# yisol/IDM-VTON

Measured on NVIDIA H100. Metric: try-on images/sec @768x1024, 30 steps, CFG 2.0, higher is better.
Workload: dtype fp16

## Files before the change

idm-vton_b200/csrc/gemm.cu:

```cuda
#include "gemm_common.cuh"
#include "host.h"
#include "wgmma.cuh"

namespace vton {

enum : int { KIND_F16 = 0, KIND_F16IN_F32OUT = 1, KIND_TF32 = 2 };

template <int BN, int STAGES, bool SC>
struct SmemLayout {
  static constexpr int B_BYTES = BN * 128;
  static constexpr int STAGE_BYTES = A_BYTES + B_BYTES;
  static constexpr int LDS = BN + 4;
  static constexpr int STG_BYTES = 128 * LDS * 4;
  static constexpr int RING = STAGES * STAGE_BYTES;
  static constexpr int STG_TOTAL = (SC ? 2 : 1) * STG_BYTES;
  static constexpr int BAR_OFFSET = RING > STG_TOTAL ? RING : STG_TOTAL;
  static constexpr int TOTAL = BAR_OFFSET + 256 + 1024;
};

constexpr int GEMM_THREADS = 288;

template <int BN, int STAGES, bool GEGLU, bool SC, int KIND>
__global__ void __launch_bounds__(GEMM_THREADS, 1)
gemm_conv_kernel(const __grid_constant__ CUtensorMap tmA, const __grid_constant__ CUtensorMap tmB,
                 const __grid_constant__ CUtensorMap tmS0, const __grid_constant__ CUtensorMap tmS1,
                 const __grid_constant__ CUtensorMap tmBs, const GemmParams p) {
  using L = SmemLayout<BN, STAGES, SC>;
  constexpr int KBK = KIND == KIND_TF32 ? 32 : 64;
  extern __shared__ uint8_t smem_raw[];
  const uint32_t smem_base = (smem_u32(smem_raw) + 1023u) & ~1023u;
  float* stg = reinterpret_cast<float*>(smem_raw + (smem_base - smem_u32(smem_raw)));
  const uint32_t bar_base = smem_base + L::BAR_OFFSET;
  auto full_bar = [&](int s) { return bar_base + 8u * s; };
  auto empty_bar = [&](int s) { return bar_base + 8u * (STAGES + s); };

  const int warp = threadIdx.x >> 5;
  const int lane = threadIdx.x & 31;
  const int tile = blockIdx.x;
  const int n_tile = tile % p.n_tiles;
  const int m_tile = tile / p.n_tiles;
  const int n0 = n_tile * BN;
  const int total_slabs = p.slabs_main + (SC ? p.slabs_sc : 0);

  int b0 = 0, y0 = 0, x0 = 0;
  if (p.conv) {
    const int tx = m_tile % p.tiles_x;
    const int ty = (m_tile / p.tiles_x) % p.tiles_y;
    const int tb = m_tile / (p.tiles_x * p.tiles_y);
    x0 = tx * p.bw;
    y0 = ty * p.bh;
    b0 = tb * p.bb;
  }

  if (warp == 8 && lane == 0) {
    tma_prefetch_desc(&tmA);
    tma_prefetch_desc(&tmB);
    if (SC) {
      tma_prefetch_desc(&tmS0);
      tma_prefetch_desc(&tmS1);
      tma_prefetch_desc(&tmBs);
    }
    for (int s = 0; s < STAGES; ++s) {
      mbar_init(full_bar(s), 1);
      mbar_init(empty_bar(s), 2);
    }
    fence_barrier_init();
  }
  pdl_wait();
  __syncthreads();
  pdl_launch_dependents();

  if (warp == 8) {
    if (lane == 0) {
      for (int s = 0; s < total_slabs; ++s) {
        const int stage = s % STAGES;
        const uint32_t phase = (s / STAGES) & 1;
        mbar_wait(empty_bar(stage), phase ^ 1);
        const uint32_t a_dst = smem_base + stage * L::STAGE_BYTES;
        const uint32_t b_dst = a_dst + A_BYTES;
        mbar_expect_tx(full_bar(stage), L::STAGE_BYTES);
        if (s < p.slabs_main) {
          if (p.conv) {
            const int tap = s / p.cin_slabs;
            const int c0 = (s - tap * p.cin_slabs) * KBK;
            const int dy = tap / 3 - 1, dx = tap % 3 - 1;
            tma_load_4d(a_dst, &tmA, full_bar(stage), c0, x0 * p.stride + dx, y0 * p.stride + dy, b0);
            tma_load_2d(b_dst, &tmB, full_bar(stage), c0, tap * p.cout + n0);
          } else {
            tma_load_2d(a_dst, &tmA, full_bar(stage), s * KBK, m_tile * BM);
            tma_load_2d(b_dst, &tmB, full_bar(stage), s * KBK, n0);
          }
        } else {
          const int ss = s - p.slabs_main;
          if (ss < p.sc_split)
            tma_load_4d(a_dst, &tmS0, full_bar(stage), ss * BK, x0, y0, b0);
          else
            tma_load_4d(a_dst, &tmS1, full_bar(stage), (ss - p.sc_split) * BK, x0, y0, b0);
          tma_load_2d(b_dst, &tmBs, full_bar(stage), ss * BK, n0);
        }
      }
    }
    return;
  }

  const int wg = warp >> 2;
  float acc[BN / 2];
  float acc_sc[BN / 2];
  auto run_slabs = [&](float (&accr)[BN / 2], int s_begin, int s_end) {
    for (int s = s_begin; s < s_end; ++s) {
      const int stage = s % STAGES;
      mbar_wait(full_bar(stage), (s / STAGES) & 1);
      const uint32_t a_src = smem_base + stage * L::STAGE_BYTES + wg * (64 * 128);
      const uint32_t b_src = smem_base + stage * L::STAGE_BYTES + A_BYTES;
      wgmma_fence();
#pragma unroll
      for (int k = 0; k < 4; ++k) {
        const uint64_t da = make_gmma_desc_sw128(a_src + k * 32, 0, 1024);
        const uint64_t db = make_gmma_desc_sw128(b_src + k * 32, 0, 1024);
        const int scale_d = (s > s_begin || k > 0) ? 1 : 0;
        if constexpr (KIND == KIND_TF32) {
          WgmmaTF32SS<BN>::mma(accr, da, db, scale_d);
        } else {
          WgmmaF16SS<BN, 0>::mma(accr, da, db, scale_d);
        }
      }
      wgmma_commit();
      wgmma_wait<1>();
      if (s > 0 && (threadIdx.x & 127) == 0) mbar_arrive(empty_bar((s - 1) % STAGES));
    }
  };
  run_slabs(acc, 0, p.slabs_main);
  if constexpr (SC) run_slabs(acc_sc, p.slabs_main, total_slabs);
  wgmma_wait<0>();
  fence_regs(acc);
  if (SC) fence_regs(acc_sc);

  named_bar_sync(1, 256);
  {
    const int r0 = wg * 64 + ((warp & 3) << 4) + (lane >> 2);
    const int cq = (lane & 3) * 2;
#pragma unroll
    for (int i = 0; i < BN / 8; ++i) {
      *reinterpret_cast<float2*>(stg + r0 * L::LDS + i * 8 + cq) = make_float2(acc[4 * i], acc[4 * i + 1]);
      *reinterpret_cast<float2*>(stg + (r0 + 8) * L::LDS + i * 8 + cq) = make_float2(acc[4 * i + 2], acc[4 * i + 3]);
      if (SC) {
        float* s2 = stg + 128 * L::LDS;
        *reinterpret_cast<float2*>(s2 + r0 * L::LDS + i * 8 + cq) = make_float2(acc_sc[4 * i], acc_sc[4 * i + 1]);
        *reinterpret_cast<float2*>(s2 + (r0 + 8) * L::LDS + i * 8 + cq) = make_float2(acc_sc[4 * i + 2], acc_sc[4 * i + 3]);
      }
    }
  }
  named_bar_sync(1, 256);
  const int row = threadIdx.x & 127;
  const int half = threadIdx.x >> 7;
  long long out_row;
  int sample;
  map_row(p, m_tile, row, &out_row, &sample);
  const float* srow = stg + row * L::LDS;
  if (KIND == KIND_F16) {
    epilogue_store<BN, GEGLU>(p, srow, SC ? srow + 128 * L::LDS : nullptr, n_tile, out_row, sample, half, 2);
    return;
  }
  if (out_row < 0) return;
  const float* res_row = p.res_f32 ? p.res_f32 + out_row * p.N : nullptr;
#pragma unroll 1
  for (int c = half; c < BN / 32; c += 2) {
    const int ncol = n0 + c * 32;
    if (ncol >= p.N) continue;
#pragma unroll
    for (int g = 0; g < 8; ++g) {
      float4 v = *reinterpret_cast<const float4*>(srow + c * 32 + g * 4);
      if (p.bias_f32 != nullptr) {
        const float4 b4 = __ldg(reinterpret_cast<const float4*>(p.bias_f32 + ncol + g * 4));
        v.x += b4.x, v.y += b4.y, v.z += b4.z, v.w += b4.w;
      }
      if (res_row != nullptr) {
        const float4 r4 = __ldg(reinterpret_cast<const float4*>(res_row + ncol + g * 4));
        v.x += r4.x, v.y += r4.y, v.z += r4.z, v.w += r4.w;
      }
      *reinterpret_cast<float4*>(p.out_f32 + out_row * p.N + ncol + g * 4) = v;
    }
  }
}

template <int BN, int STAGES, bool GEGLU, bool SC, int KIND>
static int launch_variant(const CUtensorMap& tmA, const CUtensorMap& tmB, const CUtensorMap& tmS0,
                          const CUtensorMap& tmS1, const CUtensorMap& tmBs, const GemmParams& p, int grid,
                          cudaStream_t stream) {
  using L = SmemLayout<BN, STAGES, SC>;
  static_assert(L::TOTAL <= 227 * 1024, "shared memory budget");
  auto kern = gemm_conv_kernel<BN, STAGES, GEGLU, SC, KIND>;
  static bool configured = false;
  if (!configured) {
    VTON_CUDA(cudaFuncSetAttribute(kern, cudaFuncAttributeMaxDynamicSharedMemorySize, L::TOTAL));
    configured = true;
  }
  VTON_CUDA(launch_kernel(kern, dim3(grid), dim3(GEMM_THREADS), L::TOTAL, stream, tmA, tmB, tmS0, tmS1, tmBs, p));
  count_launch();
  return kOk;
}

void set_auto_v2(int) {}
void set_cluster4(int) {}

static int pick_bn(int N, int m_tiles, bool geglu, bool has_shortcut, int force_bn) {
  if (force_bn >= 2000) force_bn -= 2000;
  else if (force_bn >= 1000) force_bn -= 1000;
  auto usable = [&](int bn) {
    if (geglu && ((bn != 256 && bn != 128) || N % bn != 0)) return false;
    if (has_shortcut && bn > 128) return false;
    return true;
  };
  if (force_bn) {
    const bool known = force_bn == 64 || force_bn == 128 || force_bn == 160 || force_bn == 192 || force_bn == 256;
    return known && usable(force_bn) ? force_bn : 0;
  }
  const int sms = num_sms();
  const int cands[5] = {256, 192, 160, 128, 64};
  double best = 1e300;
  int best_bn = 0;
  for (int bn : cands) {
    if (!usable(bn)) continue;
    if (bn != 128 && N % bn != 0 && !(bn == 64 && N < 64)) continue;
    const long long tiles = static_cast<long long>(m_tiles) * cdiv(N, bn);
    const long long waves = (tiles + sms - 1) / sms;
    const double cost = static_cast<double>(waves) * (bn + 64);
    if (cost < best * 0.999) {
      best = cost;
      best_bn = bn;
    }
  }
  return best_bn ? best_bn : 128;
}

static int dispatch(int bn, bool geglu, const CUtensorMap& tmA, const CUtensorMap& tmB, const CUtensorMap& tmS0,
                    const CUtensorMap& tmS1, const CUtensorMap& tmBs, GemmParams& p, int m_tiles,
                    cudaStream_t stream) {
  p.n_tiles = cdiv(p.N, bn);
  const int grid = m_tiles * p.n_tiles;
  if (geglu) {
    if (bn == 128) return launch_variant<128, 6, true, false, KIND_F16>(tmA, tmB, tmS0, tmS1, tmBs, p, grid, stream);
    if (bn == 256) return launch_variant<256, 4, true, false, KIND_F16>(tmA, tmB, tmS0, tmS1, tmBs, p, grid, stream);
    set_last_error("GEGLU epilogue supports BN 128/256 only (got %d)", bn);
    return kErrUnsupported;
  }
  if (p.slabs_sc) {
    if (bn == 64) return launch_variant<64, 8, false, true, KIND_F16>(tmA, tmB, tmS0, tmS1, tmBs, p, grid, stream);
    if (bn == 128) return launch_variant<128, 6, false, true, KIND_F16>(tmA, tmB, tmS0, tmS1, tmBs, p, grid, stream);
    set_last_error("shortcut epilogue supports BN 64/128 only (got %d)", bn);
    return kErrUnsupported;
  }
  switch (bn) {
    case 64: return launch_variant<64, 8, false, false, KIND_F16>(tmA, tmB, tmS0, tmS1, tmBs, p, grid, stream);
    case 128: return launch_variant<128, 6, false, false, KIND_F16>(tmA, tmB, tmS0, tmS1, tmBs, p, grid, stream);
    case 160: return launch_variant<160, 5, false, false, KIND_F16>(tmA, tmB, tmS0, tmS1, tmBs, p, grid, stream);
    case 192: return launch_variant<192, 4, false, false, KIND_F16>(tmA, tmB, tmS0, tmS1, tmBs, p, grid, stream);
    case 256: return launch_variant<256, 4, false, false, KIND_F16>(tmA, tmB, tmS0, tmS1, tmBs, p, grid, stream);
  }
  set_last_error("unsupported BN %d", bn);
  return kErrUnsupported;
}

int gemm_f16_impl(const void* A, long long lda, const void* W, long long ldw, void* out, long long ldo, int M, int N,
                  int K, const void* bias, const void* residual, long long ldr, const void* rowvec, long long ld_rowvec,
                  int rows_per_sample, int flags, int force_bn, cudaStream_t stream) {
  const int geglu = flags & 1;
  VTON_CHECK_ARG(M > 0 && N > 0 && K > 0, "gemm: empty problem M=%d N=%d K=%d", M, N, K);
  VTON_CHECK_ARG(K % 64 == 0, "gemm: K=%d must be a multiple of 64", K);
  VTON_CHECK_ARG(N % 8 == 0 && lda % 8 == 0 && ldw % 8 == 0 && ldo % 8 == 0, "gemm: N/lda/ldw/ldo must be multiples of 8");
  VTON_CHECK_ARG(!geglu || (N % 16 == 0 && !residual && !rowvec), "gemm: bad GEGLU configuration");
  VTON_CHECK_ARG(aligned_to(out, 16) && aligned_to(bias, 16) && aligned_to(residual, 16) && aligned_to(rowvec, 16),
                 "gemm: out/bias/residual/rowvec must be 16-byte aligned");
  VTON_CHECK_ARG((!residual || ldr % 8 == 0) && (!rowvec || ld_rowvec % 8 == 0),
                 "gemm: ldr=%lld / ld_rowvec=%lld must be multiples of 8", ldr, ld_rowvec);
  const int bn = pick_bn(N, cdiv(M, BM), geglu != 0, false, force_bn);
  VTON_CHECK_ARG(bn != 0, "gemm: tile width force_bn=%d unsupported for this problem (N=%d, geglu=%d)", force_bn, N, geglu);
  VTON_CHECK_ARG(!geglu || N % bn == 0, "gemm: GEGLU needs N %% BN == 0 (N=%d, BN=%d)", N, bn);
  CUtensorMap tmA, tmB;
  {
    uint64_t dims[2] = {static_cast<uint64_t>(K), static_cast<uint64_t>(M)};
    uint64_t strides[1] = {static_cast<uint64_t>(lda) * 2};
    uint32_t box[2] = {64, 128};
    if (int e = encode_tmap_f16(&tmA, A, 2, dims, strides, box)) return e;
  }
  {
    uint64_t dims[2] = {static_cast<uint64_t>(K), static_cast<uint64_t>(N)};
    uint64_t strides[1] = {static_cast<uint64_t>(ldw) * 2};
    uint32_t box[2] = {64, static_cast<uint32_t>(bn)};
    if (int e = encode_tmap_f16(&tmB, W, 2, dims, strides, box)) return e;
  }
  GemmParams p{};
  p.out = static_cast<__half*>(out);
  p.ld_out = static_cast<int>(ldo);
  p.M = M;
  p.N = N;
  p.bias = static_cast<const __half*>(bias);
  p.residual = static_cast<const __half*>(residual);
  p.ld_res = static_cast<int>(ldr);
  p.rowvec = static_cast<const __half*>(rowvec);
  p.ld_rowvec = static_cast<int>(ld_rowvec);
  p.rows_per_sample = rows_per_sample;
  p.slabs_main = K / 64;
  p.act_gelu = (flags & 4) ? 2 : ((flags & 2) ? 1 : 0);
  return dispatch(bn, geglu != 0, tmA, tmB, tmA, tmA, tmB, p, cdiv(M, BM), stream);
}

static void pick_box(int B, int H, int W, int* bw, int* bh, int* bb) {
  int w = 1;
  while (w < 128 && W % (w * 2) == 0) w *= 2;
  int h = 1;
  while (w * h < 128 && h * 2 <= H) h *= 2;
  *bw = w;
  *bh = h;
  *bb = 128 / (w * h);
  (void)B;
}

static int encode_nhwc(CUtensorMap* tm, const void* base, int B, int H, int W, int C, int ldc, int bw, int bh, int bb,
                       int pixel_step = 1) {
  uint64_t dims[4] = {static_cast<uint64_t>(C), static_cast<uint64_t>(W), static_cast<uint64_t>(H),
                      static_cast<uint64_t>(B)};
  uint64_t strides[3] = {static_cast<uint64_t>(ldc) * 2, static_cast<uint64_t>(W) * ldc * 2,
                         static_cast<uint64_t>(H) * W * ldc * 2};
  uint32_t box[4] = {64, static_cast<uint32_t>(bw * pixel_step), static_cast<uint32_t>(bh * pixel_step),
                     static_cast<uint32_t>(bb)};
  uint32_t estr[4] = {1, static_cast<uint32_t>(pixel_step), static_cast<uint32_t>(pixel_step), 1};
  return encode_tmap_f16(tm, base, 4, dims, strides, box, pixel_step > 1 ? estr : nullptr);
}

int conv3x3_impl(const void* x, long long ldx, int B, int Hin, int Win, int Cin, const void* w, int Cout, const void* bias,
                 const void* temb, long long ld_temb, const void* sc0, int C0, const void* sc1, int C1, const void* w_sc,
                 const void* bias_sc, const void* residual, long long ldr, void* out, long long ldo, int force_bn,
                 int stride, cudaStream_t stream) {
  VTON_CHECK_ARG(B > 0 && Hin > 0 && Win > 0, "conv3x3: empty input");
  VTON_CHECK_ARG(stride == 1 || stride == 2, "conv3x3: stride %d unsupported", stride);
  VTON_CHECK_ARG(stride == 1 || (!w_sc && !residual), "conv3x3: stride 2 has no shortcut / residual form");
  const int H = (Hin - 1) / stride + 1, W = (Win - 1) / stride + 1;
  VTON_CHECK_ARG(Cin % 64 == 0, "conv3x3: Cin=%d must be a multiple of 64 (pad channels)", Cin);
  VTON_CHECK_ARG(Cout % 8 == 0 && ldo % 8 == 0 && ldx % 8 == 0, "conv3x3: Cout/ldo/ldx must be multiples of 8");
  VTON_CHECK_ARG(C0 % 64 == 0 && C1 % 64 == 0, "conv3x3: shortcut source channels must be multiples of 64");
// ... 29 lines not shown
    }
    const int Csc = C0 + (sc1 ? C1 : 0);
    uint64_t dims[2] = {static_cast<uint64_t>(Csc), static_cast<uint64_t>(Cout)};
    uint64_t strides[1] = {static_cast<uint64_t>(Csc) * 2};
    uint32_t box[2] = {64, static_cast<uint32_t>(bn)};
    if (int e = encode_tmap_f16(&tmBs, w_sc, 2, dims, strides, box)) return e;
    p.slabs_sc = Csc / 64;
    p.sc_split = C0 / 64;
  }
  p.out = static_cast<__half*>(out);
  p.ld_out = static_cast<int>(ldo);
  p.M = B * H * W;
  p.N = Cout;
  p.bias = static_cast<const __half*>(bias);
  p.bias_sc = static_cast<const __half*>(bias_sc);
  p.residual = static_cast<const __half*>(residual);
  p.ld_res = static_cast<int>(ldr);
  p.rowvec = static_cast<const __half*>(temb);
  p.ld_rowvec = static_cast<int>(ld_temb);
  p.slabs_main = 9 * (Cin / 64);
  p.conv = 1;
  p.stride = stride;
  p.H = H;
  p.W = W;
  p.B = B;
  p.bw = bw;
  p.bh = bh;
  p.bb = bb;
  p.tiles_x = W / bw;
  p.tiles_y = cdiv(H, bh);
  p.cin_slabs = Cin / 64;
  p.cout = Cout;
  const int m_tiles = p.tiles_x * p.tiles_y * cdiv(B, bb);
  return dispatch(bn, false, tmA, tmB, tmS0, tmS1, tmBs, p, m_tiles, stream);
}

int conv3x3_f32_impl(const void* x, int B, int H, int W, int Cin, const void* w, int Cout, const void* bias,
                     const void* residual, void* out, int in_fp16, cudaStream_t stream) {
  VTON_CHECK_ARG(B > 0 && H > 0 && W > 0, "conv3x3_f32: empty input");
  VTON_CHECK_ARG(Cin % 32 == 0 && Cout % 32 == 0 && Cout >= 64, "conv3x3_f32: Cin=%d / Cout=%d must be multiples of 32 (Cout >= 64)", Cin, Cout);
  VTON_CHECK_ARG(!in_fp16 || Cin % 64 == 0, "conv3x3_f32: fp16 operands need Cin=%d to be a multiple of 64", Cin);
  VTON_CHECK_ARG(x && w && out, "conv3x3_f32: null pointer");
  const int esz = in_fp16 ? 2 : 4;
  const int bk = in_fp16 ? 64 : 32;
  int bw, bh, bb;
  pick_box(B, H, W, &bw, &bh, &bb);
  VTON_CHECK_ARG(bw * bh * bb == 128 && bw >= 8, "conv3x3_f32: W=%d H=%d cannot be tiled into 128-pixel boxes", W, H);
  const int m_tiles = (W / bw) * cdiv(H, bh) * cdiv(B, bb);
  const int bn = pick_bn(Cout, m_tiles, false, false, Cout % 256 == 0 ? 256 : 128);
  CUtensorMap tmA, tmB;
  {
    uint64_t dims[4] = {static_cast<uint64_t>(Cin), static_cast<uint64_t>(W), static_cast<uint64_t>(H), static_cast<uint64_t>(B)};
    uint64_t strides[3] = {static_cast<uint64_t>(Cin) * esz, static_cast<uint64_t>(W) * Cin * esz,
                           static_cast<uint64_t>(H) * W * Cin * esz};
    uint32_t box[4] = {static_cast<uint32_t>(bk), static_cast<uint32_t>(bw), static_cast<uint32_t>(bh), static_cast<uint32_t>(bb)};
    if (int e = in_fp16 ? encode_tmap_f16(&tmA, x, 4, dims, strides, box) : encode_tmap_f32(&tmA, x, 4, dims, strides, box)) return e;
  }
  {
    uint64_t dims[2] = {static_cast<uint64_t>(Cin), static_cast<uint64_t>(9) * Cout};
    uint64_t strides[1] = {static_cast<uint64_t>(Cin) * esz};
    uint32_t box[2] = {static_cast<uint32_t>(bk), static_cast<uint32_t>(bn)};
    if (int e = in_fp16 ? encode_tmap_f16(&tmB, w, 2, dims, strides, box) : encode_tmap_f32(&tmB, w, 2, dims, strides, box)) return e;
  }
  GemmParams p{};
  p.out_f32 = static_cast<float*>(out);
  p.bias_f32 = static_cast<const float*>(bias);
  p.res_f32 = static_cast<const float*>(residual);
  p.M = B * H * W;
  p.N = Cout;
  p.slabs_main = 9 * (Cin / bk);
  p.conv = 1;
  p.stride = 1;
  p.H = H;
  p.W = W;
  p.B = B;
  p.bw = bw;
  p.bh = bh;
  p.bb = bb;
  p.tiles_x = W / bw;
  p.tiles_y = cdiv(H, bh);
  p.cin_slabs = Cin / bk;
  p.cout = Cout;
  p.n_tiles = cdiv(Cout, bn);
  const int grid = m_tiles * p.n_tiles;
  if (in_fp16) {
    if (bn == 256) return launch_variant<256, 4, false, false, KIND_F16IN_F32OUT>(tmA, tmB, tmA, tmA, tmB, p, grid, stream);
    return launch_variant<128, 6, false, false, KIND_F16IN_F32OUT>(tmA, tmB, tmA, tmA, tmB, p, grid, stream);
  }
  if (bn == 256) return launch_variant<256, 4, false, false, KIND_TF32>(tmA, tmB, tmA, tmA, tmB, p, grid, stream);
  return launch_variant<128, 6, false, false, KIND_TF32>(tmA, tmB, tmA, tmA, tmB, p, grid, stream);
}

}
```

idm-vton_b200/csrc/gemm_common.cuh:

```cuda
#pragma once
#include "common.cuh"

namespace vton {

struct GemmParams {
  __half* out;
  int ld_out;
  int M, N;
  const __half* bias;
  const __half* bias_sc;
  const __half* residual;
  int ld_res;
  const __half* rowvec;
  int ld_rowvec;
  int rows_per_sample;
  int slabs_main;
  int slabs_sc;
  int sc_split;
  int conv;
  int H, W, B;
  int bw, bh, bb;
  int tiles_x, tiles_y;
  int cin_slabs;
  int cout;
  int n_tiles;
  int act_gelu;
  int stride;
  float* out_f32;
  const float* bias_f32;
  const float* res_f32;
};

constexpr int BM = 128;
constexpr int BK = 64;
constexpr int A_BYTES = BM * BK * 2;

__device__ __forceinline__ void map_row(const GemmParams& p, int m_tile, int r_local, long long* out_row, int* sample) {
  *out_row = -1;
  if (p.conv) {
    const int tx = m_tile % p.tiles_x;
    const int ty = (m_tile / p.tiles_x) % p.tiles_y;
    const int tb = m_tile / (p.tiles_x * p.tiles_y);
    const int lx = r_local % p.bw;
    const int ly = (r_local / p.bw) % p.bh;
    const int lb = r_local / (p.bw * p.bh);
    const int b = tb * p.bb + lb, y = ty * p.bh + ly, x = tx * p.bw + lx;
    if (b < p.B && y < p.H && x < p.W) *out_row = (static_cast<long long>(b) * p.H + y) * p.W + x;
    *sample = b;
  } else {
    const int m = m_tile * BM + r_local;
    if (m < p.M) *out_row = m;
    *sample = p.rows_per_sample > 0 ? m / p.rows_per_sample : 0;
  }
}

enum : int { EPI_BIAS = 1, EPI_ROWVEC = 2, EPI_RES = 4, EPI_RUNTIME = 8 };

__device__ __forceinline__ float gelu_erf_fast(float x) {
  const float ax = fabsf(x) * 0.70710678118654752f;
  const float t = __fdividef(1.0f, fmaf(0.3275911f, ax, 1.0f));
  float poly = fmaf(t, 1.061405429f, -1.453152027f);
  poly = fmaf(poly, t, 1.421413741f);
  poly = fmaf(poly, t, -0.284496736f);
  poly = fmaf(poly, t, 0.254829592f);
  poly *= t;
  float e;
  const float arg = -ax * ax * 1.4426950408889634f;
  asm("ex2.approx.ftz.f32 %0, %1;" : "=f"(e) : "f"(arg));
  const float erf_abs = fmaf(-poly, e, 1.0f);
  const float erf_v = copysignf(erf_abs, x);
  return 0.5f * x * (1.0f + erf_v);
}

template <int BN, bool GEGLU, int EPI>
__device__ __forceinline__ void epilogue_load(const GemmParams& p, const float* row, const float* row_sc, int c,
                                              uint32_t (&acc)[32], uint32_t (&acc2)[32]) {
#pragma unroll
  for (int i = 0; i < 32; i += 4) {
    const float4 v = *reinterpret_cast<const float4*>(row + c * 32 + i);
    acc[i] = __float_as_uint(v.x), acc[i + 1] = __float_as_uint(v.y), acc[i + 2] = __float_as_uint(v.z), acc[i + 3] = __float_as_uint(v.w);
  }
  const float* src2 = GEGLU ? row + BN / 2 : (((EPI & EPI_RUNTIME) && p.slabs_sc) ? row_sc : nullptr);
  if (src2 != nullptr) {
#pragma unroll
    for (int i = 0; i < 32; i += 4) {
      const float4 v = *reinterpret_cast<const float4*>(src2 + c * 32 + i);
      acc2[i] = __float_as_uint(v.x), acc2[i + 1] = __float_as_uint(v.y), acc2[i + 2] = __float_as_uint(v.z), acc2[i + 3] = __float_as_uint(v.w);
    }
  }
}

__device__ __forceinline__ void add_h8(float (&v)[8], const __half* src) {
  const uint4 u = *reinterpret_cast<const uint4*>(src);
  const uint32_t w[4] = {u.x, u.y, u.z, u.w};
#pragma unroll
  for (int j = 0; j < 4; ++j) {
    const float2 a = unpack_h2(w[j]);
    v[2 * j] += a.x;
    v[2 * j + 1] += a.y;
  }
}
__device__ __forceinline__ void add_u4(float (&v)[8], const uint4 u) {
  const uint32_t w[4] = {u.x, u.y, u.z, u.w};
#pragma unroll
  for (int j = 0; j < 4; ++j) {
    const float2 a = unpack_h2(w[j]);
    v[2 * j] += a.x;
    v[2 * j + 1] += a.y;
  }
}
__device__ __forceinline__ void round_add_u4(float (&v)[8], const uint4 u) {
  const uint32_t w[4] = {u.x, u.y, u.z, u.w};
#pragma unroll
  for (int j = 0; j < 4; ++j) {
    const float2 a = unpack_h2(w[j]);
    v[2 * j] = round_h(v[2 * j]) + a.x;
    v[2 * j + 1] = round_h(v[2 * j + 1]) + a.y;
  }
}
__device__ __forceinline__ void round_add_h8(float (&v)[8], const __half* src) {
  const uint4 u = *reinterpret_cast<const uint4*>(src);
  const uint32_t w[4] = {u.x, u.y, u.z, u.w};
#pragma unroll
  for (int j = 0; j < 4; ++j) {
    const float2 a = unpack_h2(w[j]);
    v[2 * j] = round_h(v[2 * j]) + a.x;
    v[2 * j + 1] = round_h(v[2 * j + 1]) + a.y;
  }
}

template <int BN, bool GEGLU, int EPI>
__device__ __forceinline__ void epilogue_math(const GemmParams& p, int n_tile, long long out_row, int sample, int c,
                                              const uint32_t (&acc)[32], const uint32_t (&acc2)[32], uint32_t (&pk)[16],
                                              const uint4* res_pre = nullptr, const uint4* bias_pre = nullptr) {
  constexpr bool RT = (EPI & EPI_RUNTIME) != 0;
  const bool has_bias = RT ? (p.bias != nullptr) : ((EPI & EPI_BIAS) != 0);
  const bool has_rowvec = RT ? (p.rowvec != nullptr) : ((EPI & EPI_ROWVEC) != 0);
  const bool has_res = RT ? (p.residual != nullptr) : ((EPI & EPI_RES) != 0);
  const int n0 = n_tile * BN;
  const int out_n0 = GEGLU ? n_tile * (BN / 2) : n0;
  const int out_N = GEGLU ? p.N / 2 : p.N;
  const __half* rowvec_row = (has_rowvec && out_row >= 0) ? p.rowvec + static_cast<long long>(sample) * p.ld_rowvec : nullptr;
  const __half* res_row = (has_res && out_row >= 0) ? p.residual + out_row * p.ld_res : nullptr;
#pragma unroll
  for (int g = 0; g < 4; ++g) {
    const int ncol = out_n0 + c * 32 + g * 8;
    const bool col_ok = ncol < out_N;
    float v[8];
#pragma unroll
    for (int j = 0; j < 8; ++j) v[j] = __uint_as_float(acc[g * 8 + j]);
    if (GEGLU) {
      const int bcol = n0 + c * 32 + g * 8;
      float gt[8];
#pragma unroll
      for (int j = 0; j < 8; ++j) gt[j] = __uint_as_float(acc2[g * 8 + j]);
      if (p.bias && col_ok) {
        add_h8(v, p.bias + bcol);
        add_h8(gt, p.bias + bcol + BN / 2);
      }
#pragma unroll
      for (int j = 0; j < 8; ++j) {
        const float hv = round_h(v[j]);
        const float gv = round_h(gt[j]);
        v[j] = hv * round_h(gelu_erf_fast(gv));
      }
    } else {
      if (bias_pre != nullptr) {
        if (has_bias) add_u4(v, bias_pre[g]);
      } else if (has_bias && col_ok) {
        add_h8(v, p.bias + ncol);
      }
      if (RT && p.act_gelu) {
#pragma unroll 1
        for (int j = 0; j < 8; ++j) {
          const float x = round_h(v[j]);
          v[j] = p.act_gelu == 2 ? __fdividef(x, 1.0f + __expf(-1.702f * x)) : gelu_erf_fast(x);
        }
      }
      if (has_rowvec && col_ok && rowvec_row != nullptr) round_add_h8(v, rowvec_row + ncol);
      if (RT && p.slabs_sc) {
        float s[8];
#pragma unroll
        for (int j = 0; j < 8; ++j) s[j] = __uint_as_float(acc2[g * 8 + j]);
        if (p.bias_sc && col_ok) add_h8(s, p.bias_sc + ncol);
#pragma unroll
        for (int j = 0; j < 8; ++j) v[j] = round_h(s[j]) + round_h(v[j]);
      }
      if (res_pre != nullptr) {
        if (has_res) round_add_u4(v, res_pre[g]);
      } else if (has_res && col_ok && res_row != nullptr) {
        round_add_h8(v, res_row + ncol);
      }
    }
    pk[g * 4 + 0] = pack_h2(v[0], v[1]);
    pk[g * 4 + 1] = pack_h2(v[2], v[3]);
    pk[g * 4 + 2] = pack_h2(v[4], v[5]);
    pk[g * 4 + 3] = pack_h2(v[6], v[7]);
  }
}

template <int BN, bool GEGLU>
__device__ __forceinline__ void epilogue_store(const GemmParams& p, const float* row, const float* row_sc, int n_tile,
                                               long long out_row, int sample, int c_first, int c_step) {
  constexpr int OUT_COLS = GEGLU ? BN / 2 : BN;
  const int out_n0 = GEGLU ? n_tile * (BN / 2) : n_tile * BN;
  const int out_N = GEGLU ? p.N / 2 : p.N;
#pragma unroll 1
  for (int c = c_first; c < OUT_COLS / 32; c += c_step) {
    if (out_row < 0 || out_n0 + c * 32 >= out_N) continue;
    uint32_t acc[32], acc2[32];
    uint32_t pk[16];
    epilogue_load<BN, GEGLU, EPI_RUNTIME>(p, row, row_sc, c, acc, acc2);
    epilogue_math<BN, GEGLU, EPI_RUNTIME>(p, n_tile, out_row, sample, c, acc, acc2, pk);
#pragma unroll
    for (int g = 0; g < 4; ++g) {
      const int ncol = out_n0 + c * 32 + g * 8;
      if (ncol >= out_N) continue;
      *reinterpret_cast<uint4*>(p.out + out_row * p.ld_out + ncol) =
          make_uint4(pk[g * 4], pk[g * 4 + 1], pk[g * 4 + 2], pk[g * 4 + 3]);
    }
  }
}

__device__ __forceinline__ void tma_store_2d(const CUtensorMap* m, uint32_t src, int c0, int c1) {
  asm volatile("cp.async.bulk.tensor.2d.global.shared::cta.bulk_group [%0, {%2, %3}], [%1];"
               ::"l"(reinterpret_cast<uint64_t>(m)), "r"(src), "r"(c0), "r"(c1)
               : "memory");
}
__device__ __forceinline__ void tma_store_4d(const CUtensorMap* m, uint32_t src, int c0, int c1, int c2, int c3) {
  asm volatile("cp.async.bulk.tensor.4d.global.shared::cta.bulk_group [%0, {%2, %3, %4, %5}], [%1];"
               ::"l"(reinterpret_cast<uint64_t>(m)), "r"(src), "r"(c0), "r"(c1), "r"(c2), "r"(c3)
               : "memory");
}
__device__ __forceinline__ void tma_store_commit() { asm volatile("cp.async.bulk.commit_group;" ::: "memory"); }
template <int N>
__device__ __forceinline__ void tma_store_wait_read() {
  asm volatile("cp.async.bulk.wait_group.read %0;" ::"n"(N) : "memory");
}
template <int N>
__device__ __forceinline__ void tma_store_wait_all() {
  asm volatile("cp.async.bulk.wait_group %0;" ::"n"(N) : "memory");
}

}
```

Baseline: 0.8038.

## Make GEMM kernel persistent with register-direct epilogue and setmaxnreg warp specialization

Converts the GEMM/conv kernel into a persistent kernel that launches at most one CTA per SM and loops over tiles, with a producer that keeps issuing TMA loads across tile boundaries. The epilogue now works straight from accumulator registers, using quad transposes and prefetched bias and residual values, instead of staging through shared memory. This removes the staging buffer and its barriers. Block size rises to 384 threads, and setmaxnreg moves registers from the producer warpgroup to the consumers. The aim is to overlap the next tile's loads with the current epilogue and to cut launch and tail costs. The trade-offs are register pressure and less coalesced stores.

```diff
diff --git a/idm-vton_b200/csrc/gemm.cu b/idm-vton_b200/csrc/gemm.cu
--- a/idm-vton_b200/csrc/gemm.cu
+++ b/idm-vton_b200/csrc/gemm.cu
@@ -6,51 +6,34 @@
 
 enum : int { KIND_F16 = 0, KIND_F16IN_F32OUT = 1, KIND_TF32 = 2 };
 
-template <int BN, int STAGES, bool SC>
+template <int BN, int STAGES>
 struct SmemLayout {
   static constexpr int B_BYTES = BN * 128;
   static constexpr int STAGE_BYTES = A_BYTES + B_BYTES;
-  static constexpr int LDS = BN + 4;
-  static constexpr int STG_BYTES = 128 * LDS * 4;
-  static constexpr int RING = STAGES * STAGE_BYTES;
-  static constexpr int STG_TOTAL = (SC ? 2 : 1) * STG_BYTES;
-  static constexpr int BAR_OFFSET = RING > STG_TOTAL ? RING : STG_TOTAL;
+  static constexpr int BAR_OFFSET = STAGES * STAGE_BYTES;
   static constexpr int TOTAL = BAR_OFFSET + 256 + 1024;
 };
 
-constexpr int GEMM_THREADS = 288;
+constexpr int GEMM_THREADS = 384;
+constexpr int GEMM_PRODUCER_REGS = 40;
+constexpr int GEMM_CONSUMER_REGS = 232;
 
 template <int BN, int STAGES, bool GEGLU, bool SC, int KIND>
 __global__ void __launch_bounds__(GEMM_THREADS, 1)
 gemm_conv_kernel(const __grid_constant__ CUtensorMap tmA, const __grid_constant__ CUtensorMap tmB,
                  const __grid_constant__ CUtensorMap tmS0, const __grid_constant__ CUtensorMap tmS1,
                  const __grid_constant__ CUtensorMap tmBs, const GemmParams p) {
-  using L = SmemLayout<BN, STAGES, SC>;
+  using L = SmemLayout<BN, STAGES>;
   constexpr int KBK = KIND == KIND_TF32 ? 32 : 64;
   extern __shared__ uint8_t smem_raw[];
   const uint32_t smem_base = (smem_u32(smem_raw) + 1023u) & ~1023u;
-  float* stg = reinterpret_cast<float*>(smem_raw + (smem_base - smem_u32(smem_raw)));
   const uint32_t bar_base = smem_base + L::BAR_OFFSET;
   auto full_bar = [&](int s) { return bar_base + 8u * s; };
   auto empty_bar = [&](int s) { return bar_base + 8u * (STAGES + s); };
 
   const int warp = threadIdx.x >> 5;
   const int lane = threadIdx.x & 31;
-  const int tile = blockIdx.x;
-  const int n_tile = tile % p.n_tiles;
-  const int m_tile = tile / p.n_tiles;
-  const int n0 = n_tile * BN;
   const int total_slabs = p.slabs_main + (SC ? p.slabs_sc : 0);
-
-  int b0 = 0, y0 = 0, x0 = 0;
-  if (p.conv) {
-    const int tx = m_tile % p.tiles_x;
-    const int ty = (m_tile / p.tiles_x) % p.tiles_y;
-    const int tb = m_tile / (p.tiles_x * p.tiles_y);
-    x0 = tx * p.bw;
-    y0 = ty * p.bh;
-    b0 = tb * p.bb;
-  }
 
   if (warp == 8 && lane == 0) {
     tma_prefetch_desc(&tmA);
@@ -70,46 +53,64 @@
   __syncthreads();
   pdl_launch_dependents();
 
-  if (warp == 8) {
-    if (lane == 0) {
-      for (int s = 0; s < total_slabs; ++s) {
-        const int stage = s % STAGES;
-        const uint32_t phase = (s / STAGES) & 1;
-        mbar_wait(empty_bar(stage), phase ^ 1);
-        const uint32_t a_dst = smem_base + stage * L::STAGE_BYTES;
-        const uint32_t b_dst = a_dst + A_BYTES;
-        mbar_expect_tx(full_bar(stage), L::STAGE_BYTES);
-        if (s < p.slabs_main) {
-          if (p.conv) {
-            const int tap = s / p.cin_slabs;
-            const int c0 = (s - tap * p.cin_slabs) * KBK;
-            const int dy = tap / 3 - 1, dx = tap % 3 - 1;
-            tma_load_4d(a_dst, &tmA, full_bar(stage), c0, x0 * p.stride + dx, y0 * p.stride + dy, b0);
-            tma_load_2d(b_dst, &tmB, full_bar(stage), c0, tap * p.cout + n0);
+  if (warp >= 8) {
+    setmaxnreg_dec<GEMM_PRODUCER_REGS>();
+    if (warp == 8 && lane == 0) {
+      uint32_t it = 0;
+      for (int tile = blockIdx.x; tile < p.total_tiles; tile += gridDim.x) {
+        const int n0 = (tile % p.n_tiles) * BN;
+        const int m_tile = tile / p.n_tiles;
+        int b0 = 0, y0 = 0, x0 = 0;
+        if (p.conv) {
+          x0 = (m_tile % p.tiles_x) * p.bw;
+          y0 = ((m_tile / p.tiles_x) % p.tiles_y) * p.bh;
+          b0 = (m_tile / (p.tiles_x * p.tiles_y)) * p.bb;
+        }
+        for (int s = 0; s < total_slabs; ++s, ++it) {
+          const int stage = it % STAGES;
+          const uint32_t phase = (it / STAGES) & 1;
+          mbar_wait(empty_bar(stage), phase ^ 1);
+          const uint32_t a_dst = smem_base + stage * L::STAGE_BYTES;
+          const uint32_t b_dst = a_dst + A_BYTES;
+          mbar_expect_tx(full_bar(stage), L::STAGE_BYTES);
+          if (s < p.slabs_main) {
+            if (p.conv) {
+              const int tap = s / p.cin_slabs;
+              const int c0 = (s - tap * p.cin_slabs) * KBK;
+              const int dy = tap / 3 - 1, dx = tap % 3 - 1;
+              tma_load_4d(a_dst, &tmA, full_bar(stage), c0, x0 * p.stride + dx, y0 * p.stride + dy, b0);
+              tma_load_2d(b_dst, &tmB, full_bar(stage), c0, tap * p.cout + n0);
+            } else {
+              tma_load_2d(a_dst, &tmA, full_bar(stage), s * KBK, m_tile * BM);
+              tma_load_2d(b_dst, &tmB, full_bar(stage), s * KBK, n0);
+            }
           } else {
-            tma_load_2d(a_dst, &tmA, full_bar(stage), s * KBK, m_tile * BM);
-            tma_load_2d(b_dst, &tmB, full_bar(stage), s * KBK, n0);
+            const int ss = s - p.slabs_main;
+            if (ss < p.sc_split)
+              tma_load_4d(a_dst, &tmS0, full_bar(stage), ss * BK, x0, y0, b0);
+            else
+              tma_load_4d(a_dst, &tmS1, full_bar(stage), (ss - p.sc_split) * BK, x0, y0, b0);
+            tma_load_2d(b_dst, &tmBs, full_bar(stage), ss * BK, n0);
           }
-        } else {
-          const int ss = s - p.slabs_main;
-          if (ss < p.sc_split)
-            tma_load_4d(a_dst, &tmS0, full_bar(stage), ss * BK, x0, y0, b0);
-          else
-            tma_load_4d(a_dst, &tmS1, full_bar(stage), (ss - p.sc_split) * BK, x0, y0, b0);
-          tma_load_2d(b_dst, &tmBs, full_bar(stage), ss * BK, n0);
         }
       }
     }
     return;
   }
 
+  setmaxnreg_inc<GEMM_CONSUMER_REGS>();
   const int wg = warp >> 2;
+  const int r_local = wg * 64 + ((warp & 3) << 4) + (lane >> 2);
   float acc[BN / 2];
   float acc_sc[BN / 2];
+  uint32_t it = 0;
+  auto release = [&](uint32_t slab) {
+    if ((threadIdx.x & 127) == 0) mbar_arrive(empty_bar(slab % STAGES));
+  };
   auto run_slabs = [&](float (&accr)[BN / 2], int s_begin, int s_end) {
-    for (int s = s_begin; s < s_end; ++s) {
-      const int stage = s % STAGES;
-      mbar_wait(full_bar(stage), (s / STAGES) & 1);
+    for (int s = s_begin; s < s_end; ++s, ++it) {
+      const int stage = it % STAGES;
+      mbar_wait(full_bar(stage), (it / STAGES) & 1);
       const uint32_t a_src = smem_base + stage * L::STAGE_BYTES + wg * (64 * 128);
       const uint32_t b_src = smem_base + stage * L::STAGE_BYTES + A_BYTES;
       wgmma_fence();
@@ -126,68 +127,30 @@
       }
       wgmma_commit();
       wgmma_wait<1>();
-      if (s > 0 && (threadIdx.x & 127) == 0) mbar_arrive(empty_bar((s - 1) % STAGES));
+      if (s > 0) release(it - 1);
     }
   };
-  run_slabs(acc, 0, p.slabs_main);
-  if constexpr (SC) run_slabs(acc_sc, p.slabs_main, total_slabs);
-  wgmma_wait<0>();
-  fence_regs(acc);
-  if (SC) fence_regs(acc_sc);
-
-  named_bar_sync(1, 256);
-  {
-    const int r0 = wg * 64 + ((warp & 3) << 4) + (lane >> 2);
-    const int cq = (lane & 3) * 2;
-#pragma unroll
-    for (int i = 0; i < BN / 8; ++i) {
-      *reinterpret_cast<float2*>(stg + r0 * L::LDS + i * 8 + cq) = make_float2(acc[4 * i], acc[4 * i + 1]);
-      *reinterpret_cast<float2*>(stg + (r0 + 8) * L::LDS + i * 8 + cq) = make_float2(acc[4 * i + 2], acc[4 * i + 3]);
-      if (SC) {
-        float* s2 = stg + 128 * L::LDS;
-        *reinterpret_cast<float2*>(s2 + r0 * L::LDS + i * 8 + cq) = make_float2(acc_sc[4 * i], acc_sc[4 * i + 1]);
-        *reinterpret_cast<float2*>(s2 + (r0 + 8) * L::LDS + i * 8 + cq) = make_float2(acc_sc[4 * i + 2], acc_sc[4 * i + 3]);
-      }
-    }
-  }
-  named_bar_sync(1, 256);
-  const int row = threadIdx.x & 127;
-  const int half = threadIdx.x >> 7;
-  long long out_row;
-  int sample;
-  map_row(p, m_tile, row, &out_row, &sample);
-  const float* srow = stg + row * L::LDS;
-  if (KIND == KIND_F16) {
-    epilogue_store<BN, GEGLU>(p, srow, SC ? srow + 128 * L::LDS : nullptr, n_tile, out_row, sample, half, 2);
-    return;
-  }
-  if (out_row < 0) return;
-  const float* res_row = p.res_f32 ? p.res_f32 + out_row * p.N : nullptr;
-#pragma unroll 1
-  for (int c = half; c < BN / 32; c += 2) {
-    const int ncol = n0 + c * 32;
-    if (ncol >= p.N) continue;
-#pragma unroll
-    for (int g = 0; g < 8; ++g) {
-      float4 v = *reinterpret_cast<const float4*>(srow + c * 32 + g * 4);
-      if (p.bias_f32 != nullptr) {
-        const float4 b4 = __ldg(reinterpret_cast<const float4*>(p.bias_f32 + ncol + g * 4));
-        v.x += b4.x, v.y += b4.y, v.z += b4.z, v.w += b4.w;
-      }
-      if (res_row != nullptr) {
-        const float4 r4 = __ldg(reinterpret_cast<const float4*>(res_row + ncol + g * 4));
-        v.x += r4.x, v.y += r4.y, v.z += r4.z, v.w += r4.w;
-      }
-      *reinterpret_cast<float4*>(p.out_f32 + out_row * p.N + ncol + g * 4) = v;
+  for (int tile = blockIdx.x; tile < p.total_tiles; tile += gridDim.x) {
+    EpilogueF16<BN, GEGLU, SC> epi;
+    if constexpr (KIND == KIND_F16) epi.begin(p, tile / p.n_tiles, tile % p.n_tiles, r_local);
+    run_slabs(acc, 0, p.slabs_main);
+    if constexpr (SC) run_slabs(acc_sc, p.slabs_main, total_slabs);
+    wgmma_wait<0>();
+    fence_regs(acc);
+    if (SC) fence_regs(acc_sc);
+    release(it - 1);
+    if constexpr (KIND == KIND_F16) {
+      epi.finish(p, acc, acc_sc);
+    } else {
+      epilogue_f32<BN>(p, tile / p.n_tiles, tile % p.n_tiles, r_local, acc);
     }
   }
 }
 
 template <int BN, int STAGES, bool GEGLU, bool SC, int KIND>
 static int launch_variant(const CUtensorMap& tmA, const CUtensorMap& tmB, const CUtensorMap& tmS0,
-                          const CUtensorMap& tmS1, const CUtensorMap& tmBs, const GemmParams& p, int grid,
-                          cudaStream_t stream) {
-  using L = SmemLayout<BN, STAGES, SC>;
+                          const CUtensorMap& tmS1, const CUtensorMap& tmBs, const GemmParams& p, cudaStream_t stream) {
+  using L = SmemLayout<BN, STAGES>;
   static_assert(L::TOTAL <= 227 * 1024, "shared memory budget");
   auto kern = gemm_conv_kernel<BN, STAGES, GEGLU, SC, KIND>;
   static bool configured = false;
@@ -195,6 +158,7 @@
     VTON_CUDA(cudaFuncSetAttribute(kern, cudaFuncAttributeMaxDynamicSharedMemorySize, L::TOTAL));
     configured = true;
   }
+  const int grid = p.total_tiles < num_sms() ? p.total_tiles : num_sms();
   VTON_CUDA(launch_kernel(kern, dim3(grid), dim3(GEMM_THREADS), L::TOTAL, stream, tmA, tmB, tmS0, tmS1, tmBs, p));
   count_launch();
   return kOk;
@@ -237,25 +201,25 @@
                     const CUtensorMap& tmS1, const CUtensorMap& tmBs, GemmParams& p, int m_tiles,
                     cudaStream_t stream) {
   p.n_tiles = cdiv(p.N, bn);
-  const int grid = m_tiles * p.n_tiles;
+  p.total_tiles = m_tiles * p.n_tiles;
   if (geglu) {
-    if (bn == 128) return launch_variant<128, 6, true, false, KIND_F16>(tmA, tmB, tmS0, tmS1, tmBs, p, grid, stream);
-    if (bn == 256) return launch_variant<256, 4, true, false, KIND_F16>(tmA, tmB, tmS0, tmS1, tmBs, p, grid, stream);
+    if (bn == 128) return launch_variant<128, 6, true, false, KIND_F16>(tmA, tmB, tmS0, tmS1, tmBs, p, stream);
+    if (bn == 256) return launch_variant<256, 4, true, false, KIND_F16>(tmA, tmB, tmS0, tmS1, tmBs, p, stream);
     set_last_error("GEGLU epilogue supports BN 128/256 only (got %d)", bn);
     return kErrUnsupported;
   }
   if (p.slabs_sc) {
-    if (bn == 64) return launch_variant<64, 8, false, true, KIND_F16>(tmA, tmB, tmS0, tmS1, tmBs, p, grid, stream);
-    if (bn == 128) return launch_variant<128, 6, false, true, KIND_F16>(tmA, tmB, tmS0, tmS1, tmBs, p, grid, stream);
+    if (bn == 64) return launch_variant<64, 8, false, true, KIND_F16>(tmA, tmB, tmS0, tmS1, tmBs, p, stream);
+    if (bn == 128) return launch_variant<128, 6, false, true, KIND_F16>(tmA, tmB, tmS0, tmS1, tmBs, p, stream);
     set_last_error("shortcut epilogue supports BN 64/128 only (got %d)", bn);
     return kErrUnsupported;
   }
   switch (bn) {
-    case 64: return launch_variant<64, 8, false, false, KIND_F16>(tmA, tmB, tmS0, tmS1, tmBs, p, grid, stream);
-    case 128: return launch_variant<128, 6, false, false, KIND_F16>(tmA, tmB, tmS0, tmS1, tmBs, p, grid, stream);
-    case 160: return launch_variant<160, 5, false, false, KIND_F16>(tmA, tmB, tmS0, tmS1, tmBs, p, grid, stream);
-    case 192: return launch_variant<192, 4, false, false, KIND_F16>(tmA, tmB, tmS0, tmS1, tmBs, p, grid, stream);
-    case 256: return launch_variant<256, 4, false, false, KIND_F16>(tmA, tmB, tmS0, tmS1, tmBs, p, grid, stream);
+    case 64: return launch_variant<64, 8, false, false, KIND_F16>(tmA, tmB, tmS0, tmS1, tmBs, p, stream);
+    case 128: return launch_variant<128, 6, false, false, KIND_F16>(tmA, tmB, tmS0, tmS1, tmBs, p, stream);
+    case 160: return launch_variant<160, 5, false, false, KIND_F16>(tmA, tmB, tmS0, tmS1, tmBs, p, stream);
+    case 192: return launch_variant<192, 4, false, false, KIND_F16>(tmA, tmB, tmS0, tmS1, tmBs, p, stream);
+    case 256: return launch_variant<256, 4, false, false, KIND_F16>(tmA, tmB, tmS0, tmS1, tmBs, p, stream);
   }
   set_last_error("unsupported BN %d", bn);
   return kErrUnsupported;
@@ -451,13 +415,13 @@
   p.cin_slabs = Cin / bk;
   p.cout = Cout;
   p.n_tiles = cdiv(Cout, bn);
-  const int grid = m_tiles * p.n_tiles;
+  p.total_tiles = m_tiles * p.n_tiles;
   if (in_fp16) {
-    if (bn == 256) return launch_variant<256, 4, false, false, KIND_F16IN_F32OUT>(tmA, tmB, tmA, tmA, tmB, p, grid, stream);
-    return launch_variant<128, 6, false, false, KIND_F16IN_F32OUT>(tmA, tmB, tmA, tmA, tmB, p, grid, stream);
-  }
-  if (bn == 256) return launch_variant<256, 4, false, false, KIND_TF32>(tmA, tmB, tmA, tmA, tmB, p, grid, stream);
-  return launch_variant<128, 6, false, false, KIND_TF32>(tmA, tmB, tmA, tmA, tmB, p, grid, stream);
-}
-
-}
+    if (bn == 256) return launch_variant<256, 4, false, false, KIND_F16IN_F32OUT>(tmA, tmB, tmA, tmA, tmB, p, stream);
+    return launch_variant<128, 6, false, false, KIND_F16IN_F32OUT>(tmA, tmB, tmA, tmA, tmB, p, stream);
+  }
+  if (bn == 256) return launch_variant<256, 4, false, false, KIND_TF32>(tmA, tmB, tmA, tmA, tmB, p, stream);
+  return launch_variant<128, 6, false, false, KIND_TF32>(tmA, tmB, tmA, tmA, tmB, p, stream);
+}
+
+}
diff --git a/idm-vton_b200/csrc/gemm_common.cuh b/idm-vton_b200/csrc/gemm_common.cuh
--- a/idm-vton_b200/csrc/gemm_common.cuh
+++ b/idm-vton_b200/csrc/gemm_common.cuh
@@ -24,6 +24,7 @@
   int cin_slabs;
   int cout;
   int n_tiles;
+  int total_tiles;
   int act_gelu;
   int stride;
   float* out_f32;
@@ -54,8 +55,6 @@
   }
 }
 
-enum : int { EPI_BIAS = 1, EPI_ROWVEC = 2, EPI_RES = 4, EPI_RUNTIME = 8 };
-
 __device__ __forceinline__ float gelu_erf_fast(float x) {
   const float ax = fabsf(x) * 0.70710678118654752f;
   const float t = __fdividef(1.0f, fmaf(0.3275911f, ax, 1.0f));
@@ -72,174 +71,168 @@
   return 0.5f * x * (1.0f + erf_v);
 }
 
-template <int BN, bool GEGLU, int EPI>
-__device__ __forceinline__ void epilogue_load(const GemmParams& p, const float* row, const float* row_sc, int c,
-                                              uint32_t (&acc)[32], uint32_t (&acc2)[32]) {
-#pragma unroll
-  for (int i = 0; i < 32; i += 4) {
-    const float4 v = *reinterpret_cast<const float4*>(row + c * 32 + i);
-    acc[i] = __float_as_uint(v.x), acc[i + 1] = __float_as_uint(v.y), acc[i + 2] = __float_as_uint(v.z), acc[i + 3] = __float_as_uint(v.w);
-  }
-  const float* src2 = GEGLU ? row + BN / 2 : (((EPI & EPI_RUNTIME) && p.slabs_sc) ? row_sc : nullptr);
-  if (src2 != nullptr) {
-#pragma unroll
-    for (int i = 0; i < 32; i += 4) {
-      const float4 v = *reinterpret_cast<const float4*>(src2 + c * 32 + i);
-      acc2[i] = __float_as_uint(v.x), acc2[i + 1] = __float_as_uint(v.y), acc2[i + 2] = __float_as_uint(v.z), acc2[i + 3] = __float_as_uint(v.w);
-    }
-  }
-}
-
-__device__ __forceinline__ void add_h8(float (&v)[8], const __half* src) {
-  const uint4 u = *reinterpret_cast<const uint4*>(src);
-  const uint32_t w[4] = {u.x, u.y, u.z, u.w};
-#pragma unroll
-  for (int j = 0; j < 4; ++j) {
-    const float2 a = unpack_h2(w[j]);
-    v[2 * j] += a.x;
-    v[2 * j + 1] += a.y;
-  }
-}
-__device__ __forceinline__ void add_u4(float (&v)[8], const uint4 u) {
-  const uint32_t w[4] = {u.x, u.y, u.z, u.w};
-#pragma unroll
-  for (int j = 0; j < 4; ++j) {
-    const float2 a = unpack_h2(w[j]);
-    v[2 * j] += a.x;
-    v[2 * j + 1] += a.y;
-  }
-}
-__device__ __forceinline__ void round_add_u4(float (&v)[8], const uint4 u) {
-  const uint32_t w[4] = {u.x, u.y, u.z, u.w};
-#pragma unroll
-  for (int j = 0; j < 4; ++j) {
-    const float2 a = unpack_h2(w[j]);
-    v[2 * j] = round_h(v[2 * j]) + a.x;
-    v[2 * j + 1] = round_h(v[2 * j + 1]) + a.y;
-  }
-}
-__device__ __forceinline__ void round_add_h8(float (&v)[8], const __half* src) {
-  const uint4 u = *reinterpret_cast<const uint4*>(src);
-  const uint32_t w[4] = {u.x, u.y, u.z, u.w};
-#pragma unroll
-  for (int j = 0; j < 4; ++j) {
-    const float2 a = unpack_h2(w[j]);
-    v[2 * j] = round_h(v[2 * j]) + a.x;
-    v[2 * j + 1] = round_h(v[2 * j + 1]) + a.y;
-  }
-}
-
-template <int BN, bool GEGLU, int EPI>
-__device__ __forceinline__ void epilogue_math(const GemmParams& p, int n_tile, long long out_row, int sample, int c,
-                                              const uint32_t (&acc)[32], const uint32_t (&acc2)[32], uint32_t (&pk)[16],
-                                              const uint4* res_pre = nullptr, const uint4* bias_pre = nullptr) {
-  constexpr bool RT = (EPI & EPI_RUNTIME) != 0;
-  const bool has_bias = RT ? (p.bias != nullptr) : ((EPI & EPI_BIAS) != 0);
-  const bool has_rowvec = RT ? (p.rowvec != nullptr) : ((EPI & EPI_ROWVEC) != 0);
-  const bool has_res = RT ? (p.residual != nullptr) : ((EPI & EPI_RES) != 0);
+__device__ __forceinline__ void quad_transpose(uint32_t (&w)[4], int q) {
+  {
+    const bool odd = (q & 1) != 0;
+    const uint32_t s0 = __shfl_xor_sync(0xffffffffu, odd ? w[0] : w[1], 1);
+    const uint32_t s1 = __shfl_xor_sync(0xffffffffu, odd ? w[2] : w[3], 1);
+    if (odd) w[0] = s0, w[2] = s1;
+    else w[1] = s0, w[3] = s1;
+  }
+  {
+    const bool hi = (q & 2) != 0;
+    const uint32_t s0 = __shfl_xor_sync(0xffffffffu, hi ? w[0] : w[2], 2);
+    const uint32_t s1 = __shfl_xor_sync(0xffffffffu, hi ? w[1] : w[3], 2);
+    if (hi) w[0] = s0, w[1] = s1;
+    else w[2] = s0, w[3] = s1;
+  }
+}
+
+__device__ __forceinline__ float2 ldg_h2(const __half* src) {
+  return unpack_h2(__ldg(reinterpret_cast<const uint32_t*>(src)));
+}
+
+template <int BN, bool GEGLU, bool SC>
+struct EpilogueF16 {
+  static constexpr int OUT_COLS = GEGLU ? BN / 2 : BN;
+  static constexpr int CHUNKS = OUT_COLS / 32;
+  static constexpr bool HAS_RES = !GEGLU && !SC;
+  static constexpr int RES_AHEAD = !HAS_RES ? 1 : (CHUNKS < 4 ? CHUNKS : 4);
+
+  int q, n0, out_n0, out_N;
+  long long out_row[2];
+  int sample[2];
+  uint32_t bias[BN / 8];
+  uint32_t bias_sc[SC ? BN / 8 : 1];
+  uint4 res[2][RES_AHEAD];
+
+  __device__ __forceinline__ int own_col(int c) const { return out_n0 + (4 * c + q) * 8; }
+
+  __device__ __forceinline__ void load_res(const GemmParams& p, int c) {
+#pragma unroll
+    for (int h = 0; h < 2; ++h) {
+      uint4 u = make_uint4(0u, 0u, 0u, 0u);
+      if (p.residual && out_row[h] >= 0 && own_col(c) < out_N)
+        u = *reinterpret_cast<const uint4*>(p.residual + out_row[h] * p.ld_res + own_col(c));
+      res[h][c % RES_AHEAD] = u;
+    }
+  }
+
+  __device__ __forceinline__ void begin(const GemmParams& p, int m_tile, int n_tile, int r_local) {
+    q = threadIdx.x & 3;
+    n0 = n_tile * BN;
+    out_n0 = GEGLU ? n_tile * (BN / 2) : n0;
+    out_N = GEGLU ? p.N / 2 : p.N;
+#pragma unroll
+    for (int h = 0; h < 2; ++h) map_row(p, m_tile, r_local + 8 * h, &out_row[h], &sample[h]);
+#pragma unroll
+    for (int i = 0; i < BN / 8; ++i) {
+      const bool ok = n0 + i * 8 < p.N;
+      bias[i] = (p.bias && ok) ? __ldg(reinterpret_cast<const uint32_t*>(p.bias + n0 + i * 8 + 2 * q)) : 0u;
+      if (SC) bias_sc[i] = (p.bias_sc && ok) ? __ldg(reinterpret_cast<const uint32_t*>(p.bias_sc + n0 + i * 8 + 2 * q)) : 0u;
+    }
+    if (HAS_RES) {
+#pragma unroll
+      for (int c = 0; c < RES_AHEAD; ++c) load_res(p, c);
+    }
+  }
+
+  __device__ __forceinline__ void finish(const GemmParams& p, const float (&acc)[BN / 2], const float (&acc_sc)[BN / 2]) {
+    const __half* rowvec_row[2];
+#pragma unroll
+    for (int h = 0; h < 2; ++h)
+      rowvec_row[h] = (p.rowvec && out_row[h] >= 0) ? p.rowvec + static_cast<long long>(sample[h]) * p.ld_rowvec : nullptr;
+#pragma unroll
+    for (int c = 0; c < CHUNKS; ++c) {
+      if (out_n0 + c * 32 >= out_N) break;
+#pragma unroll
+      for (int h = 0; h < 2; ++h) {
+        uint32_t w[4];
+#pragma unroll
+        for (int g = 0; g < 4; ++g) {
+          const int i = 4 * c + g;
+          const bool col_ok = out_n0 + i * 8 < out_N;
+          float v0 = acc[4 * i + 2 * h], v1 = acc[4 * i + 2 * h + 1];
+          if (GEGLU) {
+            float g0 = acc[4 * (i + BN / 16) + 2 * h], g1 = acc[4 * (i + BN / 16) + 2 * h + 1];
+            if (p.bias && col_ok) {
+              const float2 b = unpack_h2(bias[i]), bg = unpack_h2(bias[i + BN / 16]);
+              v0 += b.x, v1 += b.y, g0 += bg.x, g1 += bg.y;
+            }
+            v0 = round_h(v0) * round_h(gelu_erf_fast(round_h(g0)));
+            v1 = round_h(v1) * round_h(gelu_erf_fast(round_h(g1)));
+          } else {
+            if (p.bias && col_ok) {
+              const float2 b = unpack_h2(bias[i]);
+              v0 += b.x, v1 += b.y;
+            }
+            if (p.act_gelu) {
+              const float x0 = round_h(v0), x1 = round_h(v1);
+              v0 = p.act_gelu == 2 ? __fdividef(x0, 1.0f + __expf(-1.702f * x0)) : gelu_erf_fast(x0);
+              v1 = p.act_gelu == 2 ? __fdividef(x1, 1.0f + __expf(-1.702f * x1)) : gelu_erf_fast(x1);
+            }
+            if (rowvec_row[h] != nullptr && col_ok) {
+              const float2 t = ldg_h2(rowvec_row[h] + n0 + i * 8 + 2 * q);
+              v0 = round_h(v0) + t.x, v1 = round_h(v1) + t.y;
+            }
+            if (SC) {
+              float s0 = acc_sc[4 * i + 2 * h], s1 = acc_sc[4 * i + 2 * h + 1];
+              if (p.bias_sc && col_ok) {
+                const float2 b = unpack_h2(bias_sc[i]);
+                s0 += b.x, s1 += b.y;
+              }
+              v0 = round_h(s0) + round_h(v0), v1 = round_h(s1) + round_h(v1);
+            }
+          }
+          w[g] = pack_h2(v0, v1);
+        }
+        quad_transpose(w, q);
+        if (out_row[h] < 0 || own_col(c) >= out_N) continue;
+        if (HAS_RES && p.residual) {
+          const uint4 u = res[h][c % RES_AHEAD];
+          const uint32_t r[4] = {u.x, u.y, u.z, u.w};
+#pragma unroll
+          for (int j = 0; j < 4; ++j) {
+            const float2 a = unpack_h2(w[j]), d = unpack_h2(r[j]);
+            w[j] = pack_h2(a.x + d.x, a.y + d.y);
+          }
+        }
+        *reinterpret_cast<uint4*>(p.out + out_row[h] * p.ld_out + own_col(c)) = make_uint4(w[0], w[1], w[2], w[3]);
+      }
+      if (HAS_RES && c + RES_AHEAD < CHUNKS) load_res(p, c + RES_AHEAD);
+    }
+  }
+};
+
+template <int BN>
+__device__ __forceinline__ void epilogue_f32(const GemmParams& p, int m_tile, int n_tile, int r_local,
+                                             const float (&acc)[BN / 2]) {
+  const int q = threadIdx.x & 3;
   const int n0 = n_tile * BN;
-  const int out_n0 = GEGLU ? n_tile * (BN / 2) : n0;
-  const int out_N = GEGLU ? p.N / 2 : p.N;
-  const __half* rowvec_row = (has_rowvec && out_row >= 0) ? p.rowvec + static_cast<long long>(sample) * p.ld_rowvec : nullptr;
-  const __half* res_row = (has_res && out_row >= 0) ? p.residual + out_row * p.ld_res : nullptr;
-#pragma unroll
-  for (int g = 0; g < 4; ++g) {
-    const int ncol = out_n0 + c * 32 + g * 8;
-    const bool col_ok = ncol < out_N;
-    float v[8];
-#pragma unroll
-    for (int j = 0; j < 8; ++j) v[j] = __uint_as_float(acc[g * 8 + j]);
-    if (GEGLU) {
-      const int bcol = n0 + c * 32 + g * 8;
-      float gt[8];
-#pragma unroll
-      for (int j = 0; j < 8; ++j) gt[j] = __uint_as_float(acc2[g * 8 + j]);
-      if (p.bias && col_ok) {
-        add_h8(v, p.bias + bcol);
-        add_h8(gt, p.bias + bcol + BN / 2);
+  long long out_row[2];
+#pragma unroll
+  for (int h = 0; h < 2; ++h) {
+    int sample;
+    map_row(p, m_tile, r_local + 8 * h, &out_row[h], &sample);
+  }
+#pragma unroll
+  for (int i = 0; i < BN / 8; ++i) {
+    if (n0 + i * 8 >= p.N) break;
+    const int ncol = n0 + i * 8 + 2 * q;
+    float2 b = make_float2(0.0f, 0.0f);
+    if (p.bias_f32 != nullptr) b = __ldg(reinterpret_cast<const float2*>(p.bias_f32 + ncol));
+#pragma unroll
+    for (int h = 0; h < 2; ++h) {
+      if (out_row[h] < 0) continue;
+      float2 v = make_float2(acc[4 * i + 2 * h], acc[4 * i + 2 * h + 1]);
+      if (p.bias_f32 != nullptr) v.x += b.x, v.y += b.y;
+      if (p.res_f32 != nullptr) {
+        const float2 r = __ldg(reinterpret_cast<const float2*>(p.res_f32 + out_row[h] * p.N + ncol));
+        v.x += r.x, v.y += r.y;
       }
-#pragma unroll
-      for (int j = 0; j < 8; ++j) {
-        const float hv = round_h(v[j]);
-        const float gv = round_h(gt[j]);
-        v[j] = hv * round_h(gelu_erf_fast(gv));
-      }
-    } else {
-      if (bias_pre != nullptr) {
-        if (has_bias) add_u4(v, bias_pre[g]);
-      } else if (has_bias && col_ok) {
-        add_h8(v, p.bias + ncol);
-      }
-      if (RT && p.act_gelu) {
-#pragma unroll 1
-        for (int j = 0; j < 8; ++j) {
-          const float x = round_h(v[j]);
-          v[j] = p.act_gelu == 2 ? __fdividef(x, 1.0f + __expf(-1.702f * x)) : gelu_erf_fast(x);
-        }
-      }
-      if (has_rowvec && col_ok && rowvec_row != nullptr) round_add_h8(v, rowvec_row + ncol);
-      if (RT && p.slabs_sc) {
-        float s[8];
-#pragma unroll
-        for (int j = 0; j < 8; ++j) s[j] = __uint_as_float(acc2[g * 8 + j]);
-        if (p.bias_sc && col_ok) add_h8(s, p.bias_sc + ncol);
-#pragma unroll
-        for (int j = 0; j < 8; ++j) v[j] = round_h(s[j]) + round_h(v[j]);
-      }
-      if (res_pre != nullptr) {
-        if (has_res) round_add_u4(v, res_pre[g]);
-      } else if (has_res && col_ok && res_row != nullptr) {
-        round_add_h8(v, res_row + ncol);
-      }
-    }
-    pk[g * 4 + 0] = pack_h2(v[0], v[1]);
-    pk[g * 4 + 1] = pack_h2(v[2], v[3]);
-    pk[g * 4 + 2] = pack_h2(v[4], v[5]);
-    pk[g * 4 + 3] = pack_h2(v[6], v[7]);
-  }
-}
-
-template <int BN, bool GEGLU>
-__device__ __forceinline__ void epilogue_store(const GemmParams& p, const float* row, const float* row_sc, int n_tile,
-                                               long long out_row, int sample, int c_first, int c_step) {
-  constexpr int OUT_COLS = GEGLU ? BN / 2 : BN;
-  const int out_n0 = GEGLU ? n_tile * (BN / 2) : n_tile * BN;
-  const int out_N = GEGLU ? p.N / 2 : p.N;
-#pragma unroll 1
-  for (int c = c_first; c < OUT_COLS / 32; c += c_step) {
-    if (out_row < 0 || out_n0 + c * 32 >= out_N) continue;
-    uint32_t acc[32], acc2[32];
-    uint32_t pk[16];
-    epilogue_load<BN, GEGLU, EPI_RUNTIME>(p, row, row_sc, c, acc, acc2);
-    epilogue_math<BN, GEGLU, EPI_RUNTIME>(p, n_tile, out_row, sample, c, acc, acc2, pk);
-#pragma unroll
-    for (int g = 0; g < 4; ++g) {
-      const int ncol = out_n0 + c * 32 + g * 8;
-      if (ncol >= out_N) continue;
-      *reinterpret_cast<uint4*>(p.out + out_row * p.ld_out + ncol) =
-          make_uint4(pk[g * 4], pk[g * 4 + 1], pk[g * 4 + 2], pk[g * 4 + 3]);
-    }
-  }
-}
-
-__device__ __forceinline__ void tma_store_2d(const CUtensorMap* m, uint32_t src, int c0, int c1) {
-  asm volatile("cp.async.bulk.tensor.2d.global.shared::cta.bulk_group [%0, {%2, %3}], [%1];"
-               ::"l"(reinterpret_cast<uint64_t>(m)), "r"(src), "r"(c0), "r"(c1)
-               : "memory");
-}
-__device__ __forceinline__ void tma_store_4d(const CUtensorMap* m, uint32_t src, int c0, int c1, int c2, int c3) {
-  asm volatile("cp.async.bulk.tensor.4d.global.shared::cta.bulk_group [%0, {%2, %3, %4, %5}], [%1];"
-               ::"l"(reinterpret_cast<uint64_t>(m)), "r"(src), "r"(c0), "r"(c1), "r"(c2), "r"(c3)
-               : "memory");
-}
-__device__ __forceinline__ void tma_store_commit() { asm volatile("cp.async.bulk.commit_group;" ::: "memory"); }
-template <int N>
-__device__ __forceinline__ void tma_store_wait_read() {
-  asm volatile("cp.async.bulk.wait_group.read %0;" ::"n"(N) : "memory");
-}
-template <int N>
-__device__ __forceinline__ void tma_store_wait_all() {
-  asm volatile("cp.async.bulk.wait_group %0;" ::"n"(N) : "memory");
-}
-
-}
+      *reinterpret_cast<float2*>(p.out_f32 + out_row[h] * p.N + ncol) = v;
+    }
+  }
+}
+
+}
```

Result: faster. 0.8336, median of 6 (+3.7%).
